# lasgroup/Model-based-policy-optimizers

Measured on AMD Instinct MI355X. Metric: model-rollout transitions/sec + SAC updates/sec, Pendulum 5-ens h=5, higher is better.
Workload: dtype f32

## Files before the change

### model-based-policy-optimizers_amd/csrc/sac.hip

```cpp
#include "common.hpp"
#include "chain_run.hpp"
#include "p2p.hpp"
#include "sac_layered.hpp"
#include <string.h>
#include <stdlib.h>
int mbpo_p2p_make_dev(const mbpo_p2p_desc *d, P2pDev *P);

#include "sac_shared.hpp"
#include "sac_lean.hpp"

struct SacChainDesc {
  int mode;
  int netid;
  int base_sel;
  int param_off;
  int x, ldx;
  int pp0, pp1, zb, hb, y, dx;
  int slab_sel;
  int slab_off;
  int tp0, tp1;
};


struct SacArgs {
// ... 272 lines not shown
      }
    } else {
      if (ph == 0) {
        const int half = nthreads / 2;
        const bool second = tid >= half;
        for (int i2 = second ? tid - half : tid; i2 < 16 * U; i2 += half) {
          const int r = i2 & 15, d = i2 >> 4, idx = r * U + d;
          const float loc = y_pi[r * ld_y + d], raw = y_pi[r * ld_y + U + d];
          if (second) {
            const float e_al = s_lpa[idx];
            ActSample sal = normal_tanh_sample(loc, raw, e_al);
            s_lpa[idx] = sal.lp;
          } else {
            const float e_ac = s_eps[idx];
            ActSample sac = normal_tanh_sample(loc, raw, e_ac);
            s_lp[idx] = sac.lp;
            s_eps[idx] = e_ac;
            s_a[idx] = sac.a;
            s_sig[idx] = sac.sigma;
            s_raw[idx] = raw;
            s_qin[r * ld_xu + X + d] = sac.a;
          }
        }
      } else if (ph == 1) {
        float l_al = 0.f, l_ac = 0.f;
        if (tid < 16) {
          const int r = tid;
          const bool ok = row0 + r < B;
          float lp_al = 0.f, lp_ac = 0.f;
          for (int d = 0; d < U; ++d) {
            lp_al += s_lpa[r * U + d];
            lp_ac += s_lp[r * U + d];
          }
          l_al = ok ? alpha * (-lp_al - A.target_entropy) : 0.f;
          const float q0 = y_q1[r * ld_y], q1 = y_q2[r * ld_y];
          const float mq = fminf(q0, q1);
          l_ac = ok ? (alpha * lp_ac - mq) : 0.f;
          float g0 = 0.f, g1 = 0.f;
          if (ok) {
            if (q0 < q1) g0 = -invB;
            else if (q1 < q0) g1 = -invB;
            else g0 = g1 = -0.5f * invB;
          }
          if (A.jvp) {
            const float dLda = g0 * s_dx[r * ld_xu] + g1 * s_dx[(16 + r) * ld_xu];
            const float a = s_a[r], sg = s_sig[r], eps = s_eps[r], raw = s_raw[r];
            const float gz = dLda * (1.f - a * a) + alpha * invB * 2.f * a;
            const float gsig = gz * eps - alpha * invB / sg;
            s_dy[r * ld_y] = ok ? gz : 0.f;
            s_dy[r * ld_y + 1] = ok ? gsig * fast_sigmoid(raw) : 0.f;
          } else {
            s_dy[r * ld_y] = g0;
            s_dy[(16 + r) * ld_y] = g1;
          }
        }
        if (wave == 0) {
          const float al = wave_sum64(l_al), ac = wave_sum64(l_ac);
          if (tid == 0) {
            A.slab_ex[tile * 4 + 1] = ac;
            A.slab_ex[tile * 4 + 2] = al;
          }
        }
      } else if (ph == 2 && !A.jvp) {
        for (int i2 = tid; i2 < 16 * U; i2 += nthreads) {
          const int r = i2 & 15, d = i2 >> 4, idx = r * U + d;
          const bool ok = row0 + r < B;
          const float a = s_a[idx], sg = s_sig[idx], eps = s_eps[idx], raw = s_raw[idx];
          const float dLda = s_dx[r * ld_xu + X + d] + s_dx[(16 + r) * ld_xu + X + d];
          const float gz = dLda * (1.f - a * a) + alpha * invB * 2.f * a;
          const float gsig = gz * eps - alpha * invB / sg;
          s_dy[r * ld_y + d] = ok ? gz : 0.f;
          s_dy[r * ld_y + U + d] = ok ? gsig * fast_sigmoid(raw) : 0.f;
        }
      }
    }
    __syncthreads();
    if (ph == -1) {
      {
        const unsigned int seq_issued = qw0.x, seq_resolved = qw0.y;
        const bool odd = (seq_issued & 1u) == 0u;
        const float q0 = __uint_as_float(odd ? qw1.y : qw0.z), q1 = __uint_as_float(odd ? qw1.z : qw0.w), q2 = __uint_as_float(odd ? qw1.w : qw1.x);
        const float lim = (A.opt.max_norm / A.opt.grad_scale) * (A.opt.max_norm / A.opt.grad_scale) * 0.9998f;
        maybe_clip = seq_issued != seq_resolved && !(q0 < lim && q1 < lim && q2 < lim);
      }
      if (blockIdx.x == 0 && tid == 0) {
        const unsigned int slot = qw0.x & 1u;
        A.opt.slot_word[0] = slot;
        float *q = reinterpret_cast<float *>(A.opt.seq) + 2 + 3 * slot;
        q[0] = 0.f; q[1] = 0.f; q[2] = 0.f;
        A.step_count_rw[0] = count_in + 1.0f;
        if (A.p2p_epoch) {
          A.p2p_epoch[0] = ep0_in + 1u;
          A.p2p_epoch[1] = ep1_in + A.p2p_blocks;
        }
      }
    }

    SAC_STAMP(2 * ph + 4);
  }
  };
  run_phases(log_alpha_top);
  if (!maybe_clip) return;
  sac_group_norms(A.opt, s_gn, tid_);
  __syncthreads();
  if (s_gn[0] < A.opt.max_norm && s_gn[1] < A.opt.max_norm && s_gn[2] < A.opt.max_norm) return;
  if (blockIdx.x == 0 && tid_ == 0) A.opt.seq[SAC_CTL_CLIP_EVENTS] += 1u;
  sac_clip_fixup(A.opt, s_gn, opaque(tid_), nthreads);
  __threadfence();
  __syncthreads();
  run_phases(A.log_alpha[0]);
}

struct SacReduceArgs {
  const float *slab_pi, *slab_q, *slab_ex;
  int n_tiles, P, Q2, B;
  float *grads, *metrics, *metrics_accum, *ss_part, *step_count;
  unsigned int *seq;
};

__device__ __forceinline__ void group_sumsq(float g, int i, int P, int Q2, int NP, float *ss_part, float *quick = nullptr,
                                            float blk_lim = 0.f) {
  __shared__ float s_ss[3][4];
  const int tid = threadIdx.x, lane = tid & 63, wave = tid >> 6;
  const float gg = (i < NP) ? g * g : 0.f;
  const int grp = (i < P) ? 0 : (i < P + Q2 ? 1 : 2);
  float v0 = wave_sum64(grp == 0 ? gg : 0.f), v1 = wave_sum64(grp == 1 ? gg : 0.f), v2 = wave_sum64(grp == 2 ? gg : 0.f);
  if (lane == 0) {
    s_ss[0][wave] = v0;
    s_ss[1][wave] = v1;
    s_ss[2][wave] = v2;
  }
  __syncthreads();
  if (tid < 3) {
    const float part = s_ss[tid][0] + s_ss[tid][1] + s_ss[tid][2] + s_ss[tid][3];
    ss_part[blockIdx.x * 3 + tid] = part;
  }
  if (quick && tid == 0) {
    float tot = 0.f;
#pragma unroll
    for (int k = 0; k < 3; ++k) tot += s_ss[k][0] + s_ss[k][1] + s_ss[k][2] + s_ss[k][3];
    if (!(tot < blk_lim)) quick[0] = __builtin_inff();
  }
}

__global__ void __launch_bounds__(256) k_sac_reduce(SacReduceArgs A) {
  const int NP = A.P + A.Q2 + 1;
  const int i = blockIdx.x * 256 + threadIdx.x;
  const unsigned int seq_issued = (i == NP - 1) ? A.seq[0] : 0u;
  float g = 0.f;
  if (i < A.P) {
    g = slab_sum<16>(A.slab_pi, A.P, A.n_tiles, i);
  } else if (i < A.P + A.Q2) {
    const int j = i - A.P;
    g = slab_sum<16>(A.slab_q, A.Q2, A.n_tiles, j);
  } else if (i == NP - 1) {
    const float ce = slab_sum<16>(A.slab_ex, 4, A.n_tiles, 0) + slab_sum<16>(A.slab_ex, 4, A.n_tiles, 3), ac = slab_sum<16>(A.slab_ex, 4, A.n_tiles, 1),
                al = slab_sum<16>(A.slab_ex, 4, A.n_tiles, 2);
    const float invB = 1.0f / (float)A.B;
    g = al * invB;
    const float m0 = 0.5f * ce * (0.5f * invB), m1 = ac * invB, m2 = al * invB;
    A.metrics[0] = m0;
    A.metrics[1] = m1;
    A.seq[1] = seq_issued;
    A.metrics[2] = m2;
    if (A.metrics_accum) {
      const float a0 = A.metrics_accum[0], a1 = A.metrics_accum[1], a2 = A.metrics_accum[2], a4 = A.metrics_accum[4];
      A.metrics_accum[0] = a0 + m0;
      A.metrics_accum[1] = a1 + m1;
      A.metrics_accum[2] = a2 + m2;
      A.metrics_accum[4] = a4 + 1.0f;
    }
  }
  if (i < NP) A.grads[i] = g;
  group_sumsq(g, i, A.P, A.Q2, NP, A.ss_part);
}

__global__ void __launch_bounds__(256) k_sac_reduce_push(SacReduceArgs A, P2pDev X) {
  const int NP = A.P + A.Q2 + 1;
  const int i = blockIdx.x * 256 + threadIdx.x;
  const unsigned epoch = X.epoch[0];
  const unsigned int seq_issued = (i == NP - 1) ? A.seq[0] : 0u;
  float g = 0.f;
  if (i < A.P) {
    g = slab_sum<16>(A.slab_pi, A.P, A.n_tiles, i);
  } else if (i < A.P + A.Q2) {
    const int j = i - A.P;
    g = slab_sum<16>(A.slab_q, A.Q2, A.n_tiles, j);
  } else if (i == NP - 1) {
    const float ce = slab_sum<16>(A.slab_ex, 4, A.n_tiles, 0) + slab_sum<16>(A.slab_ex, 4, A.n_tiles, 3), ac = slab_sum<16>(A.slab_ex, 4, A.n_tiles, 1),
                al = slab_sum<16>(A.slab_ex, 4, A.n_tiles, 2);
    const float invB = 1.0f / (float)A.B;
    g = al * invB;
    const float m0 = 0.5f * ce * (0.5f * invB), m1 = ac * invB, m2 = al * invB;
    A.metrics[0] = m0;
    A.metrics[1] = m1;
    A.seq[1] = seq_issued;
    A.metrics[2] = m2;
    if (A.metrics_accum) {
      const float a0 = A.metrics_accum[0], a1 = A.metrics_accum[1], a2 = A.metrics_accum[2], a4 = A.metrics_accum[4];
      A.metrics_accum[0] = a0 + m0;
      A.metrics_accum[1] = a1 + m1;
      A.metrics_accum[2] = a2 + m2;
      A.metrics_accum[4] = a4 + 1.0f;
    }
  }
  p2p_push(X, epoch, i, NP, g);
}

__global__ void __launch_bounds__(256) k_sac_gather(P2pDev X, float *grads, int P, int Q2, float *ss_part) {
  const int NP = P + Q2 + 1;
  const int i = blockIdx.x * 256 + threadIdx.x;
  const unsigned epoch = X.epoch[0];
  const bool ok = p2p_wait(X, X.epoch[1]);
  float g = 0.f;
  if (i < NP) {
    g = ok ? p2p_sum(X, epoch, i) : NAN;
    grads[i] = g;
  }
  group_sumsq(g, i, P, Q2, NP, ss_part);
}

__global__ void __launch_bounds__(256) k_sac_reduce_exchange(SacReduceArgs A, P2pDev X) {
  const int NP = A.P + A.Q2 + 1;
  const int i = blockIdx.x * 256 + threadIdx.x;
  const unsigned epoch = X.epoch[0], want = X.epoch[1];
  const unsigned int seq_issued = (i == NP - 1) ? A.seq[0] : 0u;
  float g = 0.f;
  if (i < A.P) {
    g = slab_sum<16>(A.slab_pi, A.P, A.n_tiles, i);
  } else if (i < A.P + A.Q2) {
    const int j = i - A.P;
    g = slab_sum<16>(A.slab_q, A.Q2, A.n_tiles, j);
  } else if (i == NP - 1) {
    const float ce = slab_sum<16>(A.slab_ex, 4, A.n_tiles, 0) + slab_sum<16>(A.slab_ex, 4, A.n_tiles, 3), ac = slab_sum<16>(A.slab_ex, 4, A.n_tiles, 1),
                al = slab_sum<16>(A.slab_ex, 4, A.n_tiles, 2);
    const float invB = 1.0f / (float)A.B;
    g = al * invB;
    const float m0 = 0.5f * ce * (0.5f * invB), m1 = ac * invB, m2 = al * invB;
    A.metrics[0] = m0;
    A.metrics[1] = m1;
    A.seq[1] = seq_issued;
    A.metrics[2] = m2;
    if (A.metrics_accum) {
      const float a0 = A.metrics_accum[0], a1 = A.metrics_accum[1], a2 = A.metrics_accum[2], a4 = A.metrics_accum[4];
      A.metrics_accum[0] = a0 + m0;
      A.metrics_accum[1] = a1 + m1;
      A.metrics_accum[2] = a2 + m2;
      A.metrics_accum[4] = a4 + 1.0f;
    }
  }
  p2p_push(X, epoch, i, NP, g);
  const bool ok = p2p_wait(X, want);
  float gs = 0.f;
  if (i < NP) {
    gs = ok ? p2p_sum(X, epoch, i) : NAN;
    A.grads[i] = gs;
  }
  group_sumsq(gs, i, A.P, A.Q2, NP, A.ss_part);
}

__global__ void __launch_bounds__(256) k_sac_sumsq(const float *grads, int P, int Q2, float *ss_part) {
  const int NP = P + Q2 + 1;
  const int i = blockIdx.x * 256 + threadIdx.x;
  const float g = i < NP ? grads[i] : 0.f;
  group_sumsq(g, i, P, Q2, NP, ss_part);
}

__global__ void __launch_bounds__(256) k_sac_apply(SacOptArgs A) {
  __shared__ float s_scale[3];
  __shared__ float s_corr[2];
  const int tid = threadIdx.x;
  const int NP = A.P + A.Q2 + 1;
  const int i = blockIdx.x * 256 + tid;
  const bool in = i < NP;
  const float g_in = in ? A.grads[i] : 0.f, m_in = in ? A.adam_m[i] : 0.f, v_in = in ? A.adam_v[i] : 0.f, p_in = in ? A.params[i] : 0.f;
  const float count_in = A.step_count[0];
  const bool crit = in && i >= A.P && i < A.P + A.Q2;
  const float tq_in = crit ? A.target_q[i - A.P] : 0.f;
  sac_group_norms(A, s_scale, tid);
  if (tid == 192) {
    s_corr[0] = 1.f - powf(0.9f, count_in);
    s_corr[1] = 1.f - powf(0.999f, count_in);
  }
  __syncthreads();
  if (!in) return;
  const int grp = (i < A.P) ? 0 : (i < A.P + A.Q2 ? 1 : 2);
  const float gnorm = s_scale[grp];
  float g = g_in * A.grad_scale;
  if (!(gnorm < A.max_norm)) g = (g / gnorm) * A.max_norm;
  const AdamOut o = sac_adam(p_in, m_in, v_in, g, s_corr[0], s_corr[1], A.lr[grp], A.wd[grp]);
  A.adam_m[i] = o.m;
  A.adam_v[i] = o.v;
  A.params[i] = o.p;
  if (grp == 1) {
    A.target_q[i - A.P] = tq_in * A.one_minus_tau + o.p * A.tau;
  } else if (grp == 2) {
    A.metrics[3] = expf(o.p);
    if (A.metrics_accum) A.metrics_accum[3] += A.metrics[3];
    if (!(s_scale[0] < A.max_norm) || !(s_scale[1] < A.max_norm) || !(s_scale[2] < A.max_norm)) A.seq[SAC_CTL_CLIP_EVENTS] += 1u;
  }
}


template <bool EXCHANGE>
__global__ void __launch_bounds__(256) k_sac_reduce_apply(SacReduceArgs A, SacOptArgs O, P2pDev X) {
  __shared__ float s_corr[2];
  const int NP = A.P + A.Q2 + 1;
  const int tid = threadIdx.x;
  const int i = blockIdx.x * 256 + tid;
  const bool in = i < NP;
  const float m_in = in ? O.adam_m[i] : 0.f, v_in = in ? O.adam_v[i] : 0.f, p_in = in ? O.params[i] : 0.f;
  const bool crit = in && i >= A.P && i < A.P + A.Q2;
  const float tq_in = crit ? O.target_q[i - A.P] : 0.f;
  const float count = O.step_count[0];
  const bool last = (i == NP - 1);
  float acc0 = 0.f, acc1 = 0.f, acc2 = 0.f, acc3 = 0.f, acc4 = 0.f;
  unsigned int seq0 = 0u;
  if (last) {
    seq0 = O.seq[0];
    if (A.metrics_accum) {
      acc0 = A.metrics_accum[0];
      acc1 = A.metrics_accum[1];
      acc2 = A.metrics_accum[2];
      acc3 = A.metrics_accum[3];
      acc4 = A.metrics_accum[4];
    }
  }
  unsigned epoch = 0, want = 0;
  if (EXCHANGE) {
    epoch = X.epoch[0];
    want = X.epoch[1];
  }
  if (tid == 0) {
    s_corr[0] = 1.f - powf(0.9f, count);
    s_corr[1] = 1.f - powf(0.999f, count);
  }
  float g = 0.f;
  if (i < A.P) {
    g = slab_sum<16>(A.slab_pi, A.P, A.n_tiles, i);
  } else if (i < A.P + A.Q2) {
    const int j = i - A.P;
    g = slab_sum<16>(A.slab_q, A.Q2, A.n_tiles, j);
  } else if (i == NP - 1) {
    const float ce = slab_sum<16>(A.slab_ex, 4, A.n_tiles, 0) + slab_sum<16>(A.slab_ex, 4, A.n_tiles, 3), ac = slab_sum<16>(A.slab_ex, 4, A.n_tiles, 1),
                al = slab_sum<16>(A.slab_ex, 4, A.n_tiles, 2);
    const float invB = 1.0f / (float)A.B;
    g = al * invB;
    const float m0 = 0.5f * ce * (0.5f * invB), m1 = ac * invB, m2 = al * invB;
    A.metrics[0] = m0;
    A.metrics[1] = m1;
    A.metrics[2] = m2;
    if (A.metrics_accum) {
      A.metrics_accum[0] = acc0 + m0;
      A.metrics_accum[1] = acc1 + m1;
      A.metrics_accum[2] = acc2 + m2;
      A.metrics_accum[4] = acc4 + 1.0f;
    }
    O.undo_count[0] = count;
    O.undo_count[1] = acc3;
    O.seq[1] = seq0;
    O.seq[0] = seq0 + 1u;
  }
  if (EXCHANGE) {
    p2p_push(X, epoch, i, NP, g);
    const bool ok = p2p_wait(X, want);
    g = in ? (ok ? p2p_sum(X, epoch, i) : NAN) : 0.f;
  }
  if (in) A.grads[i] = g;
  group_sumsq(g, i, A.P, A.Q2, NP, A.ss_part, reinterpret_cast<float *>(O.seq) + 2 + 3 * (O.slot_word[0] & 1u),
              (O.max_norm / O.grad_scale) * (O.max_norm / O.grad_scale) * 0.9998f / (float)O.n_parts);
  if (!in) return;
  const int grp = (i < A.P) ? 0 : (i < A.P + A.Q2 ? 1 : 2);
  float *u_p = O.undo, *u_m = O.undo + NP, *u_v = O.undo + 2 * NP, *u_tq = O.undo + 3 * NP;
  u_p[i] = p_in;
  u_m[i] = m_in;
  u_v[i] = v_in;
  const AdamOut o = sac_adam(p_in, m_in, v_in, g * O.grad_scale, s_corr[0], s_corr[1], O.lr[grp], O.wd[grp]);
  O.params[i] = o.p;
  O.adam_m[i] = o.m;
  O.adam_v[i] = o.v;
  if (grp == 1) {
    u_tq[i - A.P] = tq_in;
    O.target_q[i - A.P] = tq_in * O.one_minus_tau + o.p * O.tau;
  } else if (grp == 2) {
    O.undo_count[2] = s_corr[0];
    O.undo_count[3] = s_corr[1];
    const float al = expf(o.p);
    O.metrics[3] = al;
    if (O.metrics_accum) O.metrics_accum[3] = acc3 + al;
  }
}

__global__ void __launch_bounds__(1024) k_sac_finalize(SacOptArgs O, unsigned long long *rng_dev, unsigned long long rng_inc) {
  __shared__ float s_gn[4];
  const int tid = threadIdx.x;
  if (rng_dev && tid == 0) rng_dev[1] += rng_inc;
  if (O.seq[0] == O.seq[1]) return;
  sac_group_norms(O, s_gn, tid);
  __syncthreads();
  const bool clip = !(s_gn[0] < O.max_norm) || !(s_gn[1] < O.max_norm) || !(s_gn[2] < O.max_norm);
  if (clip) {
    sac_clip_fixup(O, s_gn, tid, 1024);
    if (tid == 0) O.seq[SAC_CTL_CLIP_EVENTS] += 1u;
    __threadfence();
  }
  __syncthreads();
  if (tid == 0) O.seq[1] = O.seq[0];
}

struct SacPlan {
  MlpDev pi, q, qt;
  int P, Q, NP, n_tiles, H, LH, n_red;
  size_t lds;
  int ld_x, ld_xu, ld_h, ld_y;
  long long off_slab_pi, off_slab_q, off_slab_ex, off_ss, off_seq, off_undo, off_layered, total;
  bool layered;
};

static int sac_plan(const mbpo_sac_desc *d, SacPlan *pl, bool need_ptrs) {
  MBPO_REQUIRE(d, MBPO_ERR_ARG, "sac: null descriptor");
  MBPO_REQUIRE(d->x_dim > 0 && d->u_dim > 0 && d->batch_size > 0, MBPO_ERR_ARG, "sac: x_dim/u_dim/batch_size must be positive");
  MBPO_REQUIRE(d->row_len == 2 * d->x_dim + d->u_dim + 3, MBPO_ERR_ARG, "sac: row_len %d != 2x+u+3", d->row_len);
  MBPO_REQUIRE(d->policy_layers >= 2 && d->policy_layers <= MBPO_MAX_LAYERS && d->q_layers >= 2 && d->q_layers <= MBPO_MAX_LAYERS,
               MBPO_ERR_ARG, "sac: networks need at least one hidden layer and at most %d Dense layers", MBPO_MAX_LAYERS);
  MBPO_REQUIRE(d->policy_dims[0] == d->x_dim && d->policy_dims[d->policy_layers] == 2 * d->u_dim, MBPO_ERR_ARG,
               "sac: policy must map [x_dim] -> [2*u_dim]");
  MBPO_REQUIRE(d->q_dims[0] == d->x_dim + d->u_dim && d->q_dims[d->q_layers] == 1, MBPO_ERR_ARG,
               "sac: critic must map [x_dim+u_dim] -> [1]");
  const int Hp = same_hidden(d->policy_dims, d->policy_layers), Hq = same_hidden(d->q_dims, d->q_layers);
  pl->layered = mbpo_knob(KNOB_SAC_LAYERED) != 0 || !(Hp == Hq && (Hp == 64 || Hp == 128));
  int rc = mbpo_make_mlp_dev_from(d->policy_dims, d->policy_layers, d->policy_activation, d->params, 1, "sac.policy", &pl->pi);
  if (rc != MBPO_OK) return rc;
  pl->P = pl->pi.n_params;
  rc = mbpo_make_mlp_dev_from(d->q_dims, d->q_layers, d->q_activation, d->params, 1, "sac.q", &pl->q);
  if (rc != MBPO_OK) return rc;
  pl->Q = pl->q.n_params;
  pl->q.n_nets = 2;
  pl->q.net_stride = pl->Q;
  pl->q.params = d->params ? d->params + pl->P : nullptr;
  pl->qt = pl->q;
  pl->qt.params = d->target_q;
  pl->NP = pl->P + 2 * pl->Q + 1;
  pl->H = Hp;
  const int lhp = d->policy_layers - 1, lhq = d->q_layers - 1;
  pl->LH = lhp > lhq ? lhp : lhq;
  pl->n_tiles = (d->batch_size + 15) / 16;
  pl->n_red = (pl->NP + 255) / 256;
  pl->off_layered = 0;
  pl->ld_x = up4(d->x_dim) + 4;
  pl->ld_xu = up4(d->x_dim + d->u_dim) + 4;
  pl->ld_h = Hp + 4;
  pl->ld_y = up4(2 * d->u_dim) + 4;
  const int U = d->u_dim;
  size_t f = 16ull * up4(d->row_len) + 2ull * 16 * pl->ld_x + 2ull * 16 * pl->ld_xu + 4ull * 16 * pl->ld_h +
             (size_t)pl->LH * 4 * 16 * pl->ld_h + 5ull * 16 * pl->ld_y + 2ull * 16 * pl->ld_xu + 6ull * up4(16 * U) + 64 + 4;
  pl->lds = f * sizeof(float);
  if (!pl->layered && pl->lds > 160 * 1024) pl->layered = true;
  if (pl->layered) pl->n_tiles = 1;
  pl->off_slab_pi = 0;
  pl->off_slab_q = pl->off_slab_pi + (long long)pl->n_tiles * pl->P;
  pl->off_slab_ex = pl->off_slab_q + (long long)pl->n_tiles * 2 * pl->Q;
  pl->off_ss = pl->off_slab_ex + (long long)pl->n_tiles * 4;
  pl->off_seq = (pl->off_ss + (long long)pl->n_red * 3 + 3) & ~3LL;
  pl->off_undo = pl->off_seq + 16;
  pl->total = pl->off_undo + 3LL * pl->NP + 2LL * pl->Q;
  if (pl->layered) {
    pl->off_layered = (pl->total + 3) & ~3LL;
    pl->total = pl->off_layered + sac_layered_floats(d, pl->pi, pl->q);
  }
  if (need_ptrs) {
    MBPO_REQUIRE(d->params && d->target_q && d->adam_m && d->adam_v && d->step_count && d->grads && d->workspace && d->metrics,
                 MBPO_ERR_ARG, "sac: null state pointer");
  }
  return MBPO_OK;
}

extern "C" int64_t mbpo_sac_workspace_floats(const mbpo_sac_desc *d) {
  SacPlan pl;
  int rc = sac_plan(d, &pl, false);
  if (rc != MBPO_OK) return rc;
  return pl.total;
}

extern "C" int64_t mbpo_sac_control_offset(const mbpo_sac_desc *d) {
  SacPlan pl;
  int rc = sac_plan(d, &pl, false);
  if (rc != MBPO_OK) return rc;
  return pl.off_seq;
}

constexpr int SP64 = 4;

static void sac_chain_table(const SacPlan &pl, int D, SacArgs *A, bool split, bool jvp) {
  const int ld_x = pl.ld_x, ld_xu = pl.ld_xu, ld_h = pl.ld_h, ld_y = pl.ld_y, LH = pl.LH;
  const int T = 16 * ld_h;
  const int o_row = 0;
  const int o_sn = o_row + 16 * ((D + 3) & ~3), o_sn2 = o_sn + 16 * ld_x, o_qin = o_sn2 + 16 * ld_x, o_qin2 = o_qin + 16 * ld_xu;
  const int o_pp = o_qin2 + 16 * ld_xu, o_st0 = o_pp + 4 * T, o_y = o_st0 + 4 * LH * T, o_dy = o_y + 3 * 16 * ld_y, o_dx = o_dy + 2 * 16 * ld_y;
  const int o_st1 = o_st0 + LH * T, o_st2 = o_st0 + 2 * LH * T, o_st3 = o_st0 + 3 * LH * T;
  const int P = pl.P, Q = pl.Q;
  for (int role = 0; role < 3; ++role)
    for (int ph = 0; ph < 5; ++ph)
      for (int c = 0; c < 4; ++c) {
        SacChainDesc d;
        memset(&d, 0, sizeof(d));
        d.mode = CH_IDLE;
        d.x = d.pp0 = d.pp1 = d.zb = d.hb = d.y = d.dx = d.tp0 = d.tp1 = -1;
        d.ldx = ld_x;
        const int net = c & 1;
        if (split && role != 1) {
          const int kq = role >> 1;
          if (ph == 0 && c < 2) {
            d.mode = CH_FWD;
            if (c == 0) {
              d.netid = 0; d.param_off = 0; d.x = o_sn2; d.ldx = ld_x; d.pp0 = o_pp; d.pp1 = o_pp + T; d.y = o_y;
            } else {
              d.netid = 1; d.param_off = P + kq * Q; d.x = o_qin; d.ldx = ld_xu;
              d.zb = kq == 0 ? o_st0 : o_st2; d.hb = kq == 0 ? o_st1 : o_st3; d.y = o_y + (kq + 1) * 16 * ld_y;
            }
          } else if (ph == 1 && c < 2) {
            d.mode = CH_FWD;
            d.netid = 1; d.base_sel = 1; d.param_off = c * Q; d.x = o_qin2; d.ldx = ld_xu;
            d.pp0 = o_pp + 2 * c * T; d.pp1 = d.pp0 + T; d.y = o_y + (c + 1) * 16 * ld_y;
          } else if (ph == 2 && c < 2) {
            d.mode = c == 0 ? CH_DGRAD : CH_WGRAD;
            d.netid = 1; d.param_off = P + kq * Q; d.x = o_qin; d.ldx = ld_xu;
            d.pp0 = o_pp + 2 * kq * T; d.pp1 = d.pp0 + T; d.zb = kq ? o_st2 : o_st0; d.hb = kq ? o_st3 : o_st1;
            d.y = o_dy + kq * 16 * ld_y;
            d.slab_sel = 2; d.slab_off = kq * Q;
          }
        } else if (role == 2) {
        } else if (role == 0) {
          if (ph == 0 && c < 3) {
            d.mode = CH_FWD;
            if (c == 0) {
              d.netid = 0; d.param_off = 0; d.x = o_sn2; d.ldx = ld_x; d.pp0 = o_pp; d.pp1 = o_pp + T; d.y = o_y;
            } else {
              d.netid = 1; d.param_off = P + (c - 1) * Q; d.x = o_qin; d.ldx = ld_xu;
              d.zb = c == 1 ? o_st0 : o_st2; d.hb = c == 1 ? o_st1 : o_st3; d.y = o_y + c * 16 * ld_y;
            }
          } else if (ph == 1 && c < 2) {
            d.mode = CH_FWD;
            d.netid = 1; d.base_sel = 1; d.param_off = c * Q; d.x = o_qin2; d.ldx = ld_xu;
            d.pp0 = o_pp + 2 * c * T; d.pp1 = d.pp0 + T; d.y = o_y + (c + 1) * 16 * ld_y;
          } else if (ph == 2) {
            d.mode = c < 2 ? CH_DGRAD : CH_WGRAD;
            d.netid = 1; d.param_off = P + net * Q; d.x = o_qin; d.ldx = ld_xu;
            d.pp0 = o_pp + 2 * net * T; d.pp1 = d.pp0 + T; d.zb = net ? o_st2 : o_st0; d.hb = net ? o_st3 : o_st1;
            d.y = o_dy + net * 16 * ld_y;
            d.slab_sel = 2; d.slab_off = net * Q;
          }
        } else {
          if (ph == 0 && c == 0) {
            d.mode = CH_FWD;
            d.netid = 0; d.param_off = 0; d.x = o_sn; d.ldx = ld_x; d.zb = o_st0; d.hb = o_st1; d.y = o_y;
          } else if (ph == 1 && c < 2) {
            d.mode = CH_FWD;
            d.netid = 1; d.param_off = P + c * Q; d.x = o_qin; d.ldx = ld_xu;
            d.pp0 = o_pp + 2 * c * T; d.pp1 = d.pp0 + T; d.zb = c == 0 ? o_st2 : o_st3; d.y = o_y + (c + 1) * 16 * ld_y;
            if (jvp) {
              d.zb = -1;
              d.tp0 = c == 0 ? o_st2 : o_st3; d.tp1 = d.tp0 + T; d.dx = o_dx + c * 16 * ld_xu;
            }
          } else if (jvp && ph == 2 && c < 2) {
            d.mode = c == 0 ? CH_DGRAD : CH_WGRAD;
            d.netid = 0; d.param_off = 0; d.x = o_sn; d.ldx = ld_x; d.pp0 = o_pp; d.pp1 = o_pp + T; d.zb = o_st0; d.hb = o_st1;
            d.y = o_dy; d.slab_sel = 1; d.slab_off = 0;
          } else if (jvp) {
          } else if (ph == 2 && c < 2) {
            d.mode = CH_DGRAD;
            d.netid = 1; d.param_off = P + net * Q; d.pp0 = o_pp + 2 * net * T; d.pp1 = d.pp0 + T; d.zb = net ? o_st3 : o_st2;
            d.y = o_dy + net * 16 * ld_y; d.dx = o_dx + net * 16 * ld_xu;
          } else if (ph == 3 && c < 2) {
            d.mode = c == 0 ? CH_DGRAD : CH_WGRAD;
            d.netid = 0; d.param_off = 0; d.x = o_sn; d.ldx = ld_x; d.pp0 = o_pp; d.pp1 = o_pp + T; d.zb = o_st0; d.hb = o_st1;
            d.y = o_dy; d.slab_sel = 1; d.slab_off = 0;
          }
        }
        A->tab[role][ph][c] = d;
      }
}

static void sac_fill_opt(const mbpo_sac_desc *d, const SacPlan &pl, SacOptArgs *A) {
  A->params = d->params; A->target_q = d->target_q; A->adam_m = d->adam_m; A->adam_v = d->adam_v; A->grads = d->grads;
  A->metrics = d->metrics; A->metrics_accum = d->metrics_accum; A->step_count = d->step_count; A->ss_part = d->workspace + pl.off_ss;
  A->undo = d->workspace + pl.off_undo;
  A->seq = reinterpret_cast<unsigned int *>(d->workspace + pl.off_seq);
  A->slot_word = reinterpret_cast<unsigned int *>(d->workspace + pl.off_seq + 8);
  A->undo_count = d->workspace + pl.off_seq + 9;
  A->n_parts = pl.n_red; A->P = pl.P; A->Q2 = 2 * pl.Q;
  A->lr[0] = d->lr_policy; A->lr[1] = d->lr_q; A->lr[2] = d->lr_alpha;
  A->wd[0] = d->wd_policy; A->wd[1] = d->wd_q; A->wd[2] = d->wd_alpha;
  A->max_norm = d->max_grad_norm; A->tau = d->tau; A->one_minus_tau = (float)(1.0 - (double)d->tau); A->grad_scale = d->grad_scale;
}

static int sac_grads_impl(const mbpo_sac_desc *d, int phase_mask, void *stream, const mbpo_p2p_desc *xd = nullptr,
                          bool exchange_in_reduce = false, bool apply_in_reduce = false) {
  SacPlan pl;
  int rc = sac_plan(d, &pl, true);
  if (rc != MBPO_OK) return rc;
  MBPO_REQUIRE(d->batch, MBPO_ERR_ARG, "sac_grads: null batch");
  MBPO_REQUIRE((d->norm_mean == nullptr) == (d->norm_std == nullptr), MBPO_ERR_ARG, "sac_grads: norm_mean/norm_std mismatch");
  SacArgs A;
  A.pi = pl.pi; A.q = pl.q; A.qt = pl.qt;
  A.sh_pi = net_shape(pl.pi);
  A.sh_q = net_shape(pl.q);
  const long long split_env = mbpo_knob(KNOB_SAC_SPLIT);
  const bool wide_any = net_is_wide(A.sh_pi) || net_is_wide(A.sh_q);
  const bool split = split_env >= 0 ? split_env != 0 : !wide_any;
  A.split = split ? 1 : 0;
  const int wg_per_tile = split ? 3 : 2;
  const bool reg_path = (pl.H == 64 || split) && !wide_any && pl.LH >= 2;
  const bool jvp = d->u_dim == 1 && reg_path && mbpo_knob(KNOB_SAC_JVP) != 0;
  A.jvp = jvp ? 1 : 0;
  A.thin = (mbpo_knob(KNOB_SAC_THIN) != 0 && split && jvp && pl.H == 64 && A.sh_pi.K_in <= THIN_KMAX && A.sh_q.K_in <= THIN_KMAX &&
            A.sh_pi.N_out <= THIN_NMAX && A.sh_q.N_out <= THIN_NMAX && A.sh_pi.L >= 3 && A.sh_q.L >= 3) ? 1 : 0;
  if (!pl.layered) sac_chain_table(pl, d->row_len, &A, split, jvp);
  A.X = d->x_dim; A.U = d->u_dim; A.B = d->batch_size; A.D = d->row_len;
  A.batch = d->batch; A.norm_mean = d->norm_mean; A.norm_std = d->norm_std;
  A.log_alpha = d->params + pl.NP - 1;
  A.noise_alpha = d->noise_alpha; A.noise_critic = d->noise_critic; A.noise_actor = d->noise_actor;
  A.seed = d->seed; A.offset = d->offset; A.rng_dev = (const unsigned long long *)d->rng_dev;
  sac_fill_opt(d, pl, &A.opt);
  A.step_count_rw = d->step_count;
  A.stamps = g_sac_stamps;
  P2pDev X;
  memset(&X, 0, sizeof(X));
  A.p2p_epoch = nullptr;
  A.p2p_blocks = (unsigned)pl.n_red;
  if (xd) {
    rc = mbpo_p2p_make_dev(xd, &X);
    if (rc != MBPO_OK) return rc;
    MBPO_REQUIRE(xd->n_max >= pl.NP, MBPO_ERR_ARG, "sac_grads_p2p: exchange regions hold %lld floats, the gradient has %d",
                 (long long)xd->n_max, pl.NP);
    A.p2p_epoch = X.epoch;
  }
  A.discounting = d->discounting; A.reward_scaling = d->reward_scaling; A.target_entropy = d->target_entropy;
  A.neq = d->non_equidistant_time; A.neq_cd = d->continuous_discounting; A.neq_tl = d->min_time_between_switches;
  A.neq_tu = d->max_time_between_switches; A.neq_dt = d->env_dt;
  MBPO_REQUIRE(!A.neq || A.neq_dt > 0.f, MBPO_ERR_ARG, "sac: non_equidistant_time needs env_dt > 0");
  A.slab_pi = d->workspace + pl.off_slab_pi; A.slab_q = d->workspace + pl.off_slab_q; A.slab_ex = d->workspace + pl.off_slab_ex;
  A.ld_x = pl.ld_x; A.ld_xu = pl.ld_xu; A.ld_h = pl.ld_h; A.ld_y = pl.ld_y; A.LH = pl.LH;
  hipStream_t st = (hipStream_t)stream;
  const bool lean = mbpo_knob(KNOB_SAC_LEAN) != 0 && !pl.layered && A.thin &&
                    sac_lean_supports(d->x_dim, d->u_dim, d->policy_dims, d->policy_layers, d->policy_activation, d->q_dims, d->q_layers,
                                      d->q_activation);
  if (pl.layered) {
    if (phase_mask & 1) {
      const SacLayeredBegin bg = {d->step_count, A.opt.seq, A.opt.slot_word, A.p2p_epoch, A.p2p_blocks};
      rc = sac_layered_fwd_bwd(d, pl.pi, pl.q, pl.qt, d->workspace + pl.off_layered, A.slab_pi, A.slab_q, A.slab_ex, bg, st);
      if (rc != MBPO_OK) return rc;
    }
  } else if ((phase_mask & 1) && lean) {
    SacLeanArgs L;
    L.params = d->params; L.target_q = d->target_q; L.batch = d->batch; L.norm_mean = d->norm_mean; L.norm_std = d->norm_std;
    L.noise_alpha = d->noise_alpha; L.noise_critic = d->noise_critic; L.noise_actor = d->noise_actor;
    L.rng_dev = A.rng_dev; L.seed = A.seed; L.offset = A.offset;
    L.slab_pi = A.slab_pi; L.slab_q = A.slab_q; L.slab_ex = A.slab_ex;
    L.step_count_rw = d->step_count; L.p2p_epoch = A.p2p_epoch; L.p2p_blocks = A.p2p_blocks; L.B = d->batch_size;
    L.discounting = A.discounting; L.reward_scaling = A.reward_scaling; L.target_entropy = A.target_entropy;
    L.neq = A.neq; L.neq_cd = A.neq_cd; L.neq_tl = A.neq_tl; L.neq_tu = A.neq_tu; L.neq_dt = A.neq_dt;
    L.stamps = g_sac_stamps;
    L.pad0 = 0;
    L.opt = A.opt;
    rc = sac_lean_launch(L, d->x_dim, pl.n_tiles, stream);
    if (rc != MBPO_OK) return rc;
  } else if (phase_mask & 1) {
    const dim3 grid(wg_per_tile * pl.n_tiles);
    if (pl.H == 64) {
      if (wide_any) rc = mbpo_launch<k_sac_fwd_bwd<64, SP64, true>>(grid, 256 * SP64, pl.lds, st, "sac_grads", A);
      else if (split && A.thin) rc = mbpo_launch<k_sac_fwd_bwd<64, SP64, false, 2, true>>(grid, 128 * SP64, pl.lds, st, "sac_grads", A);
      else if (split) rc = mbpo_launch<k_sac_fwd_bwd<64, SP64, false, 2>>(grid, 128 * SP64, pl.lds, st, "sac_grads", A);
      else rc = mbpo_launch<k_sac_fwd_bwd<64, SP64, false>>(grid, 256 * SP64, pl.lds, st, "sac_grads", A);
    } else if (split && !wide_any) {
      rc = mbpo_launch<k_sac_fwd_bwd<128, 4, false, 2>>(grid, 512, pl.lds, st, "sac_grads", A);
    } else {
      rc = mbpo_launch<k_sac_fwd_bwd<128, 2, false>>(grid, 512, pl.lds, st, "sac_grads", A);
    }
    if (rc != MBPO_OK) return rc;
  }
  if (!(phase_mask & 2)) {
    MBPO_CHECK_LAUNCH("sac_grads");
    return MBPO_OK;
  }
  SacReduceArgs R;
  R.slab_pi = A.slab_pi; R.slab_q = A.slab_q; R.slab_ex = A.slab_ex;
  R.n_tiles = pl.n_tiles; R.P = pl.P; R.Q2 = 2 * pl.Q; R.B = d->batch_size;
  R.grads = d->grads; R.metrics = d->metrics; R.metrics_accum = d->metrics_accum; R.ss_part = d->workspace + pl.off_ss; R.step_count = d->step_count;
  R.seq = A.opt.seq;
  if (apply_in_reduce && pl.layered) {
    if (xd) hipLaunchKernelGGL(k_sac_reduce_exchange, dim3(pl.n_red), dim3(256), 0, st, R, X);
    else hipLaunchKernelGGL(k_sac_reduce, dim3(pl.n_red), dim3(256), 0, st, R);
// ... 102 lines not shown
```

Measured before the change: 18.58 million.

## Restructure SAC reduce-apply kernel for batched slab loads and early prefetch

Rewrites the gradient slab reduction in k_sac_reduce_apply as a branch-free loop. Each thread loads 16 tiles into registers before summing them, and the 4-column extra slab is reduced inside the last wave with lane reads (readlane). Parameter and Adam state loads, plus scalar arguments pinned into SGPRs with asm constraints, are issued before the reduction so their latency overlaps it. The aim is to hide memory latency and cut divergence in this small kernel. In exchange it adds inline asm and scheduling barriers that depend on the compiler, and it makes redundant reads for out-of-range threads.

```diff
diff --git a/model-based-policy-optimizers_amd/csrc/sac.hip b/model-based-policy-optimizers_amd/csrc/sac.hip
--- a/model-based-policy-optimizers_amd/csrc/sac.hip
+++ b/model-based-policy-optimizers_amd/csrc/sac.hip
@@ -598,92 +598,162 @@
 }
 
 
+template <int NB>
+__device__ __forceinline__ void slab_batch_load(float (&v)[NB], const float *col, long long stride, int t0, int n_tiles) {
+  if (t0 + NB <= n_tiles) {
+#pragma unroll
+    for (int k = 0; k < NB; ++k) v[k] = col[(long long)(t0 + k) * stride];
+  } else {
+#pragma unroll
+    for (int k = 0; k < NB; ++k) {
+      const int t = (t0 + k < n_tiles) ? t0 + k : n_tiles - 1;
+      v[k] = col[(long long)t * stride];
+    }
+  }
+}
+template <int NB>
+__device__ __forceinline__ float slab_batch_add(float g, const float (&v)[NB], int t0, int n_tiles) {
+  if (t0 + NB <= n_tiles) {
+#pragma unroll
+    for (int k = 0; k < NB; ++k) g += v[k];
+  } else {
+#pragma unroll
+    for (int k = 0; k < NB; ++k)
+      if (t0 + k < n_tiles) g += v[k];
+  }
+  return g;
+}
+__device__ __forceinline__ float slab_ex_load(const float *slab_ex, int t0, int n_tiles, int lane) {
+  const int w = t0 * 4 + lane, w_end = n_tiles * 4 - 1;
+  return slab_ex[w < w_end ? w : w_end];
+}
+__device__ __forceinline__ void slab_ex_add(float (&s)[4], float exv, int t0, int n_tiles) {
+  const int xi = __float_as_int(exv);
+#pragma unroll
+  for (int k = 0; k < 16; ++k) {
+    if (t0 + k < n_tiles) {
+#pragma unroll
+      for (int c = 0; c < 4; ++c) s[c] += __int_as_float(__builtin_amdgcn_readlane(xi, 4 * k + c));
+    }
+  }
+}
+
 template <bool EXCHANGE>
 __global__ void __launch_bounds__(256) k_sac_reduce_apply(SacReduceArgs A, SacOptArgs O, P2pDev X) {
   __shared__ float s_corr[2];
-  const int NP = A.P + A.Q2 + 1;
-  const int tid = threadIdx.x;
+  constexpr int NB = 16;
+  typedef __attribute__((address_space(1))) float GF;
+  typedef __attribute__((address_space(1))) unsigned int GU;
+  GF *g_slab_pi = (GF *)A.slab_pi, *g_slab_q = (GF *)A.slab_q, *g_slab_ex = (GF *)A.slab_ex, *g_grads = (GF *)A.grads,
+     *g_metrics = (GF *)A.metrics, *g_metrics_accum = (GF *)A.metrics_accum, *g_ss_part = (GF *)A.ss_part, *g_params = (GF *)O.params,
+     *g_target_q = (GF *)O.target_q, *g_adam_m = (GF *)O.adam_m, *g_adam_v = (GF *)O.adam_v, *g_undo = (GF *)O.undo,
+     *g_undo_count = (GF *)O.undo_count, *g_step_count = (GF *)O.step_count;
+  GU *g_seq = (GU *)O.seq, *g_slot_word = (GU *)O.slot_word, *g_epoch = EXCHANGE ? (GU *)X.epoch : nullptr;
+  int n_tiles = A.n_tiles, P = A.P, Q2 = A.Q2, B = A.B, n_parts = O.n_parts;
+  float lr0 = O.lr[0], lr1 = O.lr[1], lr2 = O.lr[2], wd0 = O.wd[0], wd1 = O.wd[1], wd2 = O.wd[2];
+  float max_norm = O.max_norm, grad_scale = O.grad_scale, tau = O.tau, one_minus_tau = O.one_minus_tau;
+  asm("" : "+s"(g_slab_pi), "+s"(g_slab_q), "+s"(g_slab_ex), "+s"(n_tiles), "+s"(P), "+s"(Q2), "+s"(B), "+s"(g_grads),
+               "+s"(g_metrics), "+s"(g_metrics_accum), "+s"(g_ss_part), "+s"(g_params), "+s"(g_target_q), "+s"(g_adam_m), "+s"(g_adam_v));
+  asm("" : "+s"(g_undo), "+s"(g_undo_count), "+s"(g_step_count), "+s"(g_seq), "+s"(g_slot_word), "+s"(g_epoch), "+s"(n_parts),
+               "+s"(lr0), "+s"(lr1), "+s"(lr2), "+s"(wd0), "+s"(wd1), "+s"(wd2), "+s"(max_norm), "+s"(grad_scale));
+  asm("" : "+s"(tau), "+s"(one_minus_tau));
+  const float *slab_pi = (const float *)g_slab_pi, *slab_q = (const float *)g_slab_q, *slab_ex = (const float *)g_slab_ex,
+              *step_count = (const float *)g_step_count;
+  float *grads = (float *)g_grads, *metrics = (float *)g_metrics, *metrics_accum = (float *)g_metrics_accum, *ss_part = (float *)g_ss_part,
+        *params = (float *)g_params, *target_q = (float *)g_target_q, *adam_m = (float *)g_adam_m, *adam_v = (float *)g_adam_v,
+        *undo = (float *)g_undo, *undo_count = (float *)g_undo_count;
+  unsigned int *seq = (unsigned int *)g_seq, *slot_word = (unsigned int *)g_slot_word, *x_epoch = (unsigned int *)g_epoch;
+  const int NP = P + Q2 + 1;
+  const int tid = threadIdx.x, lane = tid & 63;
   const int i = blockIdx.x * 256 + tid;
-  const bool in = i < NP;
-  const float m_in = in ? O.adam_m[i] : 0.f, v_in = in ? O.adam_v[i] : 0.f, p_in = in ? O.params[i] : 0.f;
-  const bool crit = in && i >= A.P && i < A.P + A.Q2;
-  const float tq_in = crit ? O.target_q[i - A.P] : 0.f;
-  const float count = O.step_count[0];
-  const bool last = (i == NP - 1);
-  float acc0 = 0.f, acc1 = 0.f, acc2 = 0.f, acc3 = 0.f, acc4 = 0.f;
-  unsigned int seq0 = 0u;
-  if (last) {
-    seq0 = O.seq[0];
-    if (A.metrics_accum) {
-      acc0 = A.metrics_accum[0];
-      acc1 = A.metrics_accum[1];
-      acc2 = A.metrics_accum[2];
-      acc3 = A.metrics_accum[3];
-      acc4 = A.metrics_accum[4];
-    }
-  }
+  const bool in = i < NP, last = (i == NP - 1);
+  const int grp = (i < P) ? 0 : (i < P + Q2 ? 1 : 2);
+  const bool crit = in && grp == 1;
+  const bool last_wave = __builtin_amdgcn_readfirstlane(i >> 6) == ((NP - 1) >> 6);
+
+  const float count = step_count[0];
+  const unsigned int slot = slot_word[0];
+  const unsigned int seq0 = seq[0];
+  const float *ma = metrics_accum ? metrics_accum : params;
+  const float ma0 = ma[0], ma1 = ma[1], ma2 = ma[2], ma3 = ma[3], ma4 = ma[4];
   unsigned epoch = 0, want = 0;
   if (EXCHANGE) {
-    epoch = X.epoch[0];
-    want = X.epoch[1];
-  }
-  if (tid == 0) {
-    s_corr[0] = 1.f - powf(0.9f, count);
-    s_corr[1] = 1.f - powf(0.999f, count);
-  }
-  float g = 0.f;
-  if (i < A.P) {
-    g = slab_sum<16>(A.slab_pi, A.P, A.n_tiles, i);
-  } else if (i < A.P + A.Q2) {
-    const int j = i - A.P;
-    g = slab_sum<16>(A.slab_q, A.Q2, A.n_tiles, j);
-  } else if (i == NP - 1) {
-    const float ce = slab_sum<16>(A.slab_ex, 4, A.n_tiles, 0) + slab_sum<16>(A.slab_ex, 4, A.n_tiles, 3), ac = slab_sum<16>(A.slab_ex, 4, A.n_tiles, 1),
-                al = slab_sum<16>(A.slab_ex, 4, A.n_tiles, 2);
-    const float invB = 1.0f / (float)A.B;
+    epoch = x_epoch[0];
+    want = x_epoch[1];
+  }
+  asm volatile("" ::: "memory");
+  const bool wl = in && !last;
+  const float *col = !wl ? slab_pi : (grp == 0 ? slab_pi + i : slab_q + (i - P));
+  const long long stride = (wl && grp == 1) ? Q2 : P;
+  float exv = 0.f;
+  if (last_wave) exv = slab_ex_load(slab_ex, 0, n_tiles, lane);
+  float v[NB];
+  slab_batch_load<NB>(v, col, stride, 0, n_tiles);
+  const int ic = in ? i : NP - 1, jc = crit ? i - P : 0;
+  const float p_in = params[ic], m_in = adam_m[ic], v_in = adam_v[ic], tq_in = target_q[jc];
+  asm volatile("" ::: "memory");
+  __builtin_amdgcn_sched_barrier(0);
+  if (tid == 0) s_corr[0] = 1.f - powf(0.9f, count);
+  if (tid == 64) s_corr[1] = 1.f - powf(0.999f, count);
+  __builtin_amdgcn_sched_barrier(0);
+
+  const float acc0 = ma0, acc1 = ma1, acc2 = ma2, acc3 = metrics_accum ? ma3 : 0.f, acc4 = ma4;
+  float g = slab_batch_add<NB>(0.f, v, 0, n_tiles);
+  float ex[4] = {0.f, 0.f, 0.f, 0.f};
+  if (last_wave) slab_ex_add(ex, exv, 0, n_tiles);
+  for (int t0 = NB; t0 < n_tiles; t0 += NB) {
+    if (last_wave) exv = slab_ex_load(slab_ex, t0, n_tiles, lane);
+    slab_batch_load<NB>(v, col, stride, t0, n_tiles);
+    g = slab_batch_add<NB>(g, v, t0, n_tiles);
+    if (last_wave) slab_ex_add(ex, exv, t0, n_tiles);
+  }
+  if (!wl) g = 0.f;
+  if (last) {
+    const float ce = ex[0] + ex[3], ac = ex[1], al = ex[2];
+    const float invB = 1.0f / (float)B;
     g = al * invB;
     const float m0 = 0.5f * ce * (0.5f * invB), m1 = ac * invB, m2 = al * invB;
-    A.metrics[0] = m0;
-    A.metrics[1] = m1;
-    A.metrics[2] = m2;
-    if (A.metrics_accum) {
-      A.metrics_accum[0] = acc0 + m0;
-      A.metrics_accum[1] = acc1 + m1;
-      A.metrics_accum[2] = acc2 + m2;
-      A.metrics_accum[4] = acc4 + 1.0f;
-    }
-    O.undo_count[0] = count;
-    O.undo_count[1] = acc3;
-    O.seq[1] = seq0;
-    O.seq[0] = seq0 + 1u;
+    metrics[0] = m0;
+    metrics[1] = m1;
+    metrics[2] = m2;
+    if (metrics_accum) {
+      metrics_accum[0] = acc0 + m0;
+      metrics_accum[1] = acc1 + m1;
+      metrics_accum[2] = acc2 + m2;
+      metrics_accum[4] = acc4 + 1.0f;
+    }
+    undo_count[0] = count;
+    undo_count[1] = acc3;
+    seq[1] = seq0;
+    seq[0] = seq0 + 1u;
   }
   if (EXCHANGE) {
     p2p_push(X, epoch, i, NP, g);
     const bool ok = p2p_wait(X, want);
     g = in ? (ok ? p2p_sum(X, epoch, i) : NAN) : 0.f;
   }
-  if (in) A.grads[i] = g;
-  group_sumsq(g, i, A.P, A.Q2, NP, A.ss_part, reinterpret_cast<float *>(O.seq) + 2 + 3 * (O.slot_word[0] & 1u),
-              (O.max_norm / O.grad_scale) * (O.max_norm / O.grad_scale) * 0.9998f / (float)O.n_parts);
+  if (in) grads[i] = g;
+  group_sumsq(g, i, P, Q2, NP, ss_part, reinterpret_cast<float *>(seq) + 2 + 3 * (slot & 1u),
+              (max_norm / grad_scale) * (max_norm / grad_scale) * 0.9998f / (float)n_parts);
   if (!in) return;
-  const int grp = (i < A.P) ? 0 : (i < A.P + A.Q2 ? 1 : 2);
-  float *u_p = O.undo, *u_m = O.undo + NP, *u_v = O.undo + 2 * NP, *u_tq = O.undo + 3 * NP;
+  float *u_p = undo, *u_m = undo + NP, *u_v = undo + 2 * NP, *u_tq = undo + 3 * NP;
   u_p[i] = p_in;
   u_m[i] = m_in;
   u_v[i] = v_in;
-  const AdamOut o = sac_adam(p_in, m_in, v_in, g * O.grad_scale, s_corr[0], s_corr[1], O.lr[grp], O.wd[grp]);
-  O.params[i] = o.p;
-  O.adam_m[i] = o.m;
-  O.adam_v[i] = o.v;
+  const float lr = grp == 0 ? lr0 : (grp == 1 ? lr1 : lr2), wd = grp == 0 ? wd0 : (grp == 1 ? wd1 : wd2);
+  const AdamOut o = sac_adam(p_in, m_in, v_in, g * grad_scale, s_corr[0], s_corr[1], lr, wd);
+  params[i] = o.p;
+  adam_m[i] = o.m;
+  adam_v[i] = o.v;
   if (grp == 1) {
-    u_tq[i - A.P] = tq_in;
-    O.target_q[i - A.P] = tq_in * O.one_minus_tau + o.p * O.tau;
+    u_tq[i - P] = tq_in;
+    target_q[i - P] = tq_in * one_minus_tau + o.p * tau;
   } else if (grp == 2) {
-    O.undo_count[2] = s_corr[0];
-    O.undo_count[3] = s_corr[1];
+    undo_count[2] = s_corr[0];
+    undo_count[3] = s_corr[1];
     const float al = expf(o.p);
-    O.metrics[3] = al;
-    if (O.metrics_accum) O.metrics_accum[3] = acc3 + al;
+    metrics[3] = al;
+    if (metrics_accum) metrics_accum[3] = acc3 + al;
   }
 }
 
```

After: 19.49 million (median of 6 runs). 4.9% higher.
